# apache/datafusion

Hardware: AMD Instinct MI355X
Metric: tpch_q3_hash_join_rows_per_sec (higher is better)
Workload: dtype int64 keys / decimal128 payload; 1 GPU; INNER hash-join orders⋈lineitem on o_orderkey, TPC-H SF100, Q3 payload (o_orderdate,o_shippriority,l_orderkey,l_extendedprice,l_discount), device-resident inputs; build_rows=150000000, probe_rows=599960064, output_rows=599960064, join_table=rank_map, probe=single_pass_unordered, parallelism=single GPU, exchange=none

## Files before the change

datafusion_amd/csrc/internal.hpp:

```cpp
#pragma once
#include <atomic>
#include <hip/hip_runtime.h>

#include <chrono>
#include <cstdint>
#include <cstring>
#include <map>
#include <memory>
#include <mutex>
#include <stdexcept>
#include <string>
#include <thread>
#include <vector>

#include "../../include/dfgpu.h"

namespace dfgpu {

struct Error : std::runtime_error {
  using std::runtime_error::runtime_error;
};

void set_last_error(const std::string& msg);

// ... 97 lines not shown
int64_t scan_upload_caches_bytes(int device);
Runtime& rt_of(int device);
void use_device(int device);
int current_device();
const std::vector<int>& initialised_devices();
void require_init();

struct ProfileScope {
  hipEvent_t a = nullptr, b = nullptr;
  const char* name;
  int64_t bytes;
  ProfileScope(const char* name, int64_t algorithmic_bytes);
  ~ProfileScope();
};

struct DevBuf {
  void* ptr = nullptr;
  size_t bytes = 0;
  Runtime* owner = nullptr;
  std::shared_ptr<void> foreign;
  std::atomic<uint64_t> hint{0};
  std::atomic<uint64_t> all_hit_hint{0};
  explicit DevBuf(size_t n);
  DevBuf(void* p, size_t n, std::shared_ptr<void> keep_alive) : ptr(p), bytes(n), foreign(std::move(keep_alive)) {}
  ~DevBuf();
  DevBuf(const DevBuf&) = delete;
  DevBuf& operator=(const DevBuf&) = delete;
  template <typename T>
  T* as() const { return reinterpret_cast<T*>(ptr); }
};
using BufPtr = std::shared_ptr<DevBuf>;
inline BufPtr make_buf(size_t bytes) { return std::make_shared<DevBuf>(bytes ? bytes : 1); }
BufPtr make_zero_buf(size_t bytes);

void d2h(void* dst, const void* src, size_t n);
extern std::atomic<int64_t> g_pinned_driver_allocs, g_pinned_driver_ns;
void* pinned_alloc(size_t n);
void pinned_release(void* p);
void* stage_alloc(size_t n);
template <class T> struct StageAllocator {
  using value_type = T;
  StageAllocator() = default;
  template <class U> StageAllocator(const StageAllocator<U>&) {}
  T* allocate(size_t n) { return static_cast<T*>(stage_alloc(n * sizeof(T))); }
  void deallocate(T* p, size_t) { pinned_release(p); }
  template <class U> void construct(U* p) noexcept { ::new ((void*)p) U; }
  template <class U, class... A> void construct(U* p, A&&... a) { ::new ((void*)p) U(std::forward<A>(a)...); }
  template <class U> bool operator==(const StageAllocator<U>&) const { return true; }
  template <class U> bool operator!=(const StageAllocator<U>&) const { return false; }
};
template <class T> using StageVec = std::vector<T, StageAllocator<T>>;
struct PinnedBuf {
  void* ptr = nullptr;
  size_t bytes = 0;
  explicit PinnedBuf(size_t n) : ptr(pinned_alloc(n ? n : 1)), bytes(n) {}
  ~PinnedBuf() { pinned_release(ptr); }
  PinnedBuf(const PinnedBuf&) = delete;
  PinnedBuf& operator=(const PinnedBuf&) = delete;
  template <class T> T* as() const { return reinterpret_cast<T*>(ptr); }
};
void h2d_async(void* dst, const void* src, size_t n);

inline int type_width(int t) {
  switch (t) {
    case DFGPU_INT32: case DFGPU_UINT32: case DFGPU_DATE32: return 4;
    case DFGPU_INT64: case DFGPU_UINT64: case DFGPU_FLOAT64: return 8;
// ... 166 lines not shown
```

datafusion_amd/csrc/join.hip:

```cpp
#include <thread>
#include <functional>
#include <cstdlib>

#include "device.hpp"
#include "internal.hpp"
#include "grouped.hpp"

namespace dfgpu {

Table compact_table(const Table& in, const std::vector<int>& cols, const uint64_t* mask, const uint64_t* mask_valid);
void pack_bytes_to_bitmap(const uint8_t* bytes, int64_t n, uint64_t* words);

enum TableKind : int { KIND_HASH = 0, KIND_ARRAY = 1, KIND_RANK = 2, KIND_RADIX = 3, KIND_FLAT = 4, KIND_FLAT16 = 5,
                       KIND_RETURNED = 6 };
template <int KIND> constexpr bool kind_is_flat() { return KIND == KIND_FLAT || KIND == KIND_FLAT16; }
template <int KIND> constexpr bool kind_is_direct() { return KIND == KIND_ARRAY || KIND == KIND_RANK; }

struct FlatLayout {
  int n;
  uint8_t off[MAX_KEYS];
  uint8_t width[MAX_KEYS];
  int8_t null_bit[MAX_KEYS];
};
constexpr double RANK_MAP_MIN_KEY_DENSITY = 1.0 / 256.0;
// ... 250 lines not shown
        const int head_lane = 63 - __builtin_clzll(heads & ((2ull << lane) - 1ull));
        const uint64_t before = __shfl(inc - v, head_lane, 64);
        if (ok && ((tails >> lane) & 1ull)) atomicOr(&bits[w], (unsigned long long)(inc - before));
      }
    }
    return;
  }
  const int64_t stride = (int64_t)gridDim.x * BLOCK;
  for (int64_t i0 = (int64_t)blockIdx.x * BLOCK + threadIdx.x; i0 < n; i0 += stride * BUILD_UNROLL) {
    uint64_t lo[BUILD_UNROLL];
    bool ok[BUILD_UNROLL];
#pragma unroll
    for (int j = 0; j < BUILD_UNROLL; j++) {
      int64_t i = i0 + j * stride;
      lo[j] = load_key<KT>(k, i < n ? i : n - 1);
    }
#pragma unroll
    for (int j = 0; j < BUILD_UNROLL; j++) {
      int64_t i = i0 + j * stride;
      ok[j] = i < n;
      if (HASV) ok[j] = ok[j] && bit_at(k.valid, i < n ? i : n - 1);
    }
#pragma unroll
    for (int j = 0; j < BUILD_UNROLL; j++) {
      if (!ok[j]) continue;
      const uint64_t idx = lo[j] - offset;
      const unsigned long long bit = 1ull << (idx & 63);
      (void)__hip_atomic_fetch_or(&bits[idx >> 6], bit, __ATOMIC_RELAXED, __HIP_MEMORY_SCOPE_AGENT);
    }
  }
}
typedef unsigned long long rt_u64x2 __attribute__((ext_vector_type(2)));
typedef unsigned rt_u32x4 __attribute__((ext_vector_type(4)));
template <int KT>
__device__ __forceinline__ void load_keys4(const KeyCol& k, int64_t i0, uint64_t (&out)[4]) {
  if (KT == KT_I64 && ((uintptr_t)k.data & 15) == 0) {
    const rt_u64x2* p = reinterpret_cast<const rt_u64x2*>((const uint64_t*)k.data + i0);
    const rt_u64x2 a = __builtin_nontemporal_load(p), b = __builtin_nontemporal_load(p + 1);
    out[0] = a.x; out[1] = a.y; out[2] = b.x; out[3] = b.y;
  } else if ((KT == KT_I32 || KT == KT_U32) && ((uintptr_t)k.data & 15) == 0) {
    const rt_u32x4 a = __builtin_nontemporal_load(reinterpret_cast<const rt_u32x4*>((const uint32_t*)k.data + i0));
    out[0] = KT == KT_I32 ? (uint64_t)(int64_t)(int32_t)a.x : a.x;
    out[1] = KT == KT_I32 ? (uint64_t)(int64_t)(int32_t)a.y : a.y;
    out[2] = KT == KT_I32 ? (uint64_t)(int64_t)(int32_t)a.z : a.z;
    out[3] = KT == KT_I32 ? (uint64_t)(int64_t)(int32_t)a.w : a.w;
  } else {
#pragma unroll
    for (int j = 0; j < 4; j++) out[j] = load_key<KT, true>(k, i0 + j);
  }
}
constexpr int RT_ROWS = 4096;
constexpr int RT_WIN = 1024;
constexpr int RT_LANE_ROWS = 4;
constexpr int RT_CHUNK = WAVE * RT_LANE_ROWS;
constexpr int RT_STEPS = RT_ROWS / RT_CHUNK / (BLOCK / WAVE);
template <int KT, bool VERIFY>
__global__ __launch_bounds__(BLOCK) void k_rank_tab_onepass(KeyCol k, int64_t n, uint64_t offset, uint64_t range, ulonglong2* __restrict__ tab, int* __restrict__ flag) {
  __shared__ unsigned long long s_bits[RT_WIN];
  __shared__ unsigned s_first[RT_WIN];
  constexpr int WAVES = BLOCK / WAVE;
  const unsigned lane = lane_id();
  const int wv = threadIdx.x >> 6;
  const int64_t r0 = (int64_t)blockIdx.x * RT_ROWS;
  const int64_t r1 = r0 + RT_ROWS < n ? r0 + RT_ROWS : n;
  const uint64_t n_words = (range >> 6) + 1;
  uint64_t idx[RT_STEPS][RT_LANE_ROWS], pidx[RT_STEPS];
#pragma unroll
  for (int c = 0; c < RT_STEPS; c++) {
    const int64_t i0 = r0 + (int64_t)(c * WAVES + wv) * RT_CHUNK + lane * RT_LANE_ROWS;
    if (i0 + RT_LANE_ROWS <= n) {
      load_keys4<KT>(k, i0, idx[c]);
#pragma unroll
      for (int j = 0; j < RT_LANE_ROWS; j++) idx[c][j] -= offset;
    } else {
#pragma unroll
      for (int j = 0; j < RT_LANE_ROWS; j++) idx[c][j] = load_key<KT, true>(k, i0 + j < n ? i0 + j : n - 1) - offset;
    }
    pidx[c] = 0;
    if (VERIFY) pidx[c] = load_key<KT>(k, i0 < n ? (i0 > 0 ? i0 - 1 : 0) : n - 1) - offset;
  }
  const bool tail_lane = wv == WAVES - 1 && r1 + lane < n;
// ... 305 lines not shown
template <int KIND>
__device__ __forceinline__ uint32_t chain_head(const ProbeCtx& c, int64_t p) {
  if (kind_is_flat<KIND>()) {
    uint64_t k0, k1;
    if (!flat_pack(c.pkeys, c.flat_layout, p, c.null_equals_null != 0, k0, k1)) return 0u;
    return flat_find<KIND == KIND_FLAT16>(c.flat, c.flat_shift, c.flat_mask, k0, k1, c.force_collisions != 0);
  } else if (KIND != KIND_HASH) {
    const KeyCol& k = c.pkeys.c[0];
    if (k.valid && !bit_at(k.valid, p)) return 0;
    uint64_t lo, hi;
    load_words(k, p, lo, hi);
    uint64_t idx = lo - c.am_offset;
    if (idx >= c.am_size) return 0u;
    if (KIND == KIND_ARRAY) return c.heads[idx];
    const ulonglong2 e = c.rank_tab[idx >> 6];
    const uint64_t bits = e.x;
    if (!((bits >> (idx & 63)) & 1ull)) return 0u;
    const uint32_t rank = (uint32_t)e.y + (uint32_t)__popcll(bits & ((1ull << (idx & 63)) - 1ull));
    return (c.rank_perm ? c.rank_perm[rank] : rank) + 1u;
  } else {
    bool any_null;
    uint64_t h = hash_row(c.pkeys, p, SEED_JOIN, any_null);
    if (any_null && !c.null_equals_null) return 0;
    if (c.force_collisions) h = 0;
    return c.heads[h & c.hash_mask];
  }
}
template <int KIND>
__device__ __forceinline__ bool chain_match(const ProbeCtx& c, int64_t b, int64_t p) {
  if (KIND != KIND_HASH) return true;
  return keys_equal(c.bkeys, b, c.pkeys, p, c.null_equals_null);
}

template <int KIND, int KT, int N>
__device__ __forceinline__ void lookup_words(const ProbeCtx& c, int64_t w0, int64_t np, uint32_t (&m)[N], uint64_t* raw_keys = nullptr, uint4* rec16 = nullptr,
                                             uint32_t* key_rows = nullptr ) {
  const unsigned lane = lane_id();
  if (KIND == KIND_RETURNED) {
    uint32_t d[N];
    bool ok[N];
#pragma unroll
    for (int j = 0; j < N; j++) {
      const int64_t p = ((w0 + j) << 6) + lane;
      ok[j] = p < np;
      d[j] = c.ret_dest[ok[j] ? p : np - 1];
      if (c.row_mask) ok[j] = ok[j] && ((c.row_mask[w0 + j] >> lane) & 1ull);
    }
    if (rec16 && c.ret_R == 16) {
#pragma unroll
      for (int j = 0; j < N; j++) {
        ok[j] = ok[j] && d[j] != 0xFFFFFFFFu;
        rec16[j] = reinterpret_cast<const uint4*>(c.ret_rec)[ok[j] ? d[j] : 0u];
      }
#pragma unroll
      for (int j = 0; j < N; j++) m[j] = ok[j] ? rec16[j].x : 0u;
      return;
    }
#pragma unroll
    for (int j = 0; j < N; j++) {
      ok[j] = ok[j] && d[j] != 0xFFFFFFFFu;
      m[j] = *reinterpret_cast<const uint32_t*>(c.ret_rec + (uint64_t)(ok[j] ? d[j] : 0u) * (uint64_t)c.ret_R);
    }
#pragma unroll
    for (int j = 0; j < N; j++) m[j] = ok[j] ? m[j] : 0u;
    return;
  }
// ... 33 lines not shown
      int64_t p = ((w0 + j) << 6) + lane;
      const bool live = p < np && (!c.row_mask || ((c.row_mask[w0 + j] >> lane) & 1ull));
      m[j] = live ? chain_head<KIND>(c, p) : 0u;
    }
#pragma unroll
    for (int j = 0; j < N; j++) {
      int64_t p = ((w0 + j) << 6) + lane;
      while (m[j] && !chain_match<KIND>(c, (int64_t)m[j] - 1, p)) m[j] = c.next[m[j] - 1];
    }
    return;
  }
  const KeyCol& k = c.pkeys.c[0];
  uint64_t idx[N];
  bool ok[N];
#pragma unroll
  for (int j = 0; j < N; j++) {
    int64_t p = ((w0 + j) << 6) + lane;
    ok[j] = p < np;
    idx[j] = load_key<KT>(k, ok[j] ? p : np - 1);
    if (raw_keys) raw_keys[j] = idx[j];
    idx[j] -= c.am_offset;
    if (c.row_mask) ok[j] = ok[j] && ((c.row_mask[w0 + j] >> lane) & 1ull);
  }
  if (k.valid) {
    uint64_t vw[N];
#pragma unroll
    for (int j = 0; j < N; j++) {
      int64_t p = ((w0 + j) << 6) + lane;
      vw[j] = k.valid[(p < np ? p : np - 1) >> 6];
    }
#pragma unroll
    for (int j = 0; j < N; j++) ok[j] = ok[j] && ((vw[j] >> lane) & 1ull);
  }
#pragma unroll
  for (int j = 0; j < N; j++) {
    ok[j] = ok[j] && idx[j] < c.am_size;
    if (!ok[j]) idx[j] = 0;
  }
  if (KIND == KIND_ARRAY) {
#pragma unroll
    for (int j = 0; j < N; j++) m[j] = c.heads[idx[j]];
#pragma unroll
    for (int j = 0; j < N; j++) m[j] = ok[j] ? m[j] : 0u;
  } else {
    uint64_t bits[N], pre[N];
#pragma unroll
    for (int j = 0; j < N; j++) {
      const ulonglong2 e = c.rank_tab[idx[j] >> 6];
      bits[j] = e.x;
      pre[j] = e.y;
    }
#pragma unroll
    for (int j = 0; j < N; j++) {
      const bool hit = ok[j] && ((bits[j] >> (idx[j] & 63)) & 1ull);
      const uint32_t rank = (uint32_t)pre[j] + (uint32_t)__popcll(bits[j] & ((1ull << (idx[j] & 63)) - 1ull));
      m[j] = hit ? rank + 1u : 0u;
    }
    if (c.rank_perm) {
      uint32_t row[N];
#pragma unroll
      for (int j = 0; j < N; j++) row[j] = c.rank_perm[m[j] ? m[j] - 1 : 0u];
#pragma unroll
      for (int j = 0; j < N; j++) m[j] = m[j] ? row[j] + 1u : 0u;
    }
  }
}

template <int KIND, int KT, int N, bool NT = false>
__device__ __forceinline__ void hit_words(const ProbeCtx& c, int64_t w0, int64_t np, uint64_t (&word)[N], const bool* pre = nullptr, const uint64_t* keys_in = nullptr) {
  if (KIND != KIND_RANK) {
    uint32_t m[N];
    lookup_words<KIND, KT, N>(c, w0, np, m);
#pragma unroll
    for (int j = 0; j < N; j++) word[j] = ballot64(m[j] != 0);
    return;
  }
  const unsigned lane = lane_id();
  const KeyCol& k = c.pkeys.c[0];
  uint64_t idx[N];
  bool ok[N];
#pragma unroll
  for (int j = 0; j < N; j++) {
    const int64_t p = ((w0 + j) << 6) + lane;
    ok[j] = p < np;
    idx[j] = (keys_in ? keys_in[j] : load_key<KT, NT>(k, ok[j] ? p : np - 1)) - c.am_offset;
    if (pre) ok[j] = ok[j] && pre[j];
    else if (c.row_mask) ok[j] = ok[j] && ((c.row_mask[w0 + j] >> lane) & 1ull);
  }
  if (k.valid) {
    uint64_t vw[N];
#pragma unroll
    for (int j = 0; j < N; j++) {
      const int64_t p = ((w0 + j) << 6) + lane;
      vw[j] = k.valid[(p < np ? p : np - 1) >> 6];
    }
#pragma unroll
    for (int j = 0; j < N; j++) ok[j] = ok[j] && ((vw[j] >> lane) & 1ull);
  }
// ... 497 lines not shown
        }
        const int word_of_lane = lane >> 4;
#pragma unroll
        for (int q = 0; q < 4; q++) {
          const int from = (4 * lane + q) & 63;
#pragma unroll
          for (int jj = 0; jj < 4; jj++) {
            const uint32_t t = __shfl(v[jj], from);
            if (jj == word_of_lane) o[q] = t;
          }
        }
        const int64_t row0 = ((w0 + 4 * g) << 6) + 4 * (int64_t)lane;
        uint32_t* dst = reinterpret_cast<uint32_t*>(cols.dst[cidx]) + row0;
        if (row0 + 3 < np) {
          stream_store(reinterpret_cast<uint4*>(dst), make_uint4(o[0], o[1], o[2], o[3]));
        } else {
#pragma unroll
          for (int q = 0; q < 4; q++)
            if (row0 + q < np) dst[q] = o[q];
        }
      }
      continue;
    }
#pragma unroll
    for (int j = 0; j < W; j++) {
      const int64_t d = ((w0 + j) << 6) + lane;
      if (d >= np || !m[j]) continue;
      const int64_t s = (int64_t)m[j] - 1;
      switch (width) {
        case 16: jcopy_stream<uint4>(cols.src[cidx], cols.dst[cidx], s, d, false, true); break;
        case 8: jcopy_stream<uint64_t>(cols.src[cidx], cols.dst[cidx], s, d, false, true); break;
        case 1: jcopy_stream<uint8_t>(cols.src[cidx], cols.dst[cidx], s, d, false, true); break;
      }
    }
  }
}

constexpr int EL_WORDS = 128;
constexpr int EL_WORDS_SPARSE = 1024;
constexpr int EL_CAP = 8192;
template <int KIND, int KT, int EW>
__global__ __launch_bounds__(BLOCK) void k_join_emit_listed(ProbeCtx c, JoinCopyCols cols, int64_t np, const uint64_t* __restrict__ out_words,
                                                            const uint64_t* __restrict__ tile_prefix, int tiles_per_group) {
  static_assert(EW % BLOCK == 0 || BLOCK % EW == 0, "whole words per thread");
  static_assert(EW * 64 <= 65536, "a listed row is a 16-bit index into the group");
  constexpr int WPT = EW >= BLOCK ? EW / BLOCK : 1;
  __shared__ uint64_t s_word[EW];
  __shared__ uint32_t s_off[EW];
  __shared__ uint32_t s_wsum[BLOCK / WAVE];
  __shared__ uint16_t s_row[EL_CAP];
  const int64_t n_words = (np + 63) >> 6;
  const int64_t w_base = (int64_t)blockIdx.x * EW;
  const unsigned lane = lane_id();
  const int wv = threadIdx.x >> 6;
  uint64_t w[WPT];
  uint32_t cnt = 0;
#pragma unroll
  for (int t = 0; t < WPT; t++) {
    const int i = (int)threadIdx.x * WPT + t;
    w[t] = (i < EW && w_base + i < n_words) ? out_words[w_base + i] : 0ull;
    cnt += (uint32_t)__popcll(w[t]);
  }
  const uint32_t inc = wave_inclusive_sum(cnt);
  if (lane == 63) s_wsum[wv] = inc;
#pragma unroll
  for (int t = 0; t < WPT; t++) {
// ... 1378 lines not shown
  if (fused_ok && fused_mode == FUSED_UNORDERED && np > (1 << 22) && !unclustered && !in_grouped_probe && !returned) {
    int64_t row_bytes = key_bytes / std::max<int64_t>(np, 1) + out_row_bytes;
    for (int c : pout) {
      bool is_key = false;
      for (int k : pk) is_key |= k == c;
      if (!is_key) row_bytes += type_width(probe.cols[c].field.type);
    }
    if (row_bytes * (FUSED_W * BLOCK) < 12 * 6000) fused_mode = FUSED_PLACED;
  }
  const bool one_match_path = np > 0 && (probe_side_only || fast_inner);
  const bool use_fused_now = use_fused;
  const bool pred_in_counts = lazy != nullptr && use_fused && listed && fused_mode == FUSED_PLACED && !returned && (kind == KIND_RANK || kind == KIND_ARRAY);
  if (!pred_in_counts) need_mask();
  if (row_mask || pred_in_counts) {
    DFGPU_CHECK(mask_consumed != nullptr, "probe row mask without a fallback");
    *mask_consumed = use_fused || one_match_path;
    if (!*mask_consumed) return Table{};
    ctx.row_mask = row_mask;
  }
  const bool listed_flavour = use_fused_now && listed && fused_mode == FUSED_PLACED && kind == KIND_RANK;
  if (!listed_flavour) need_tab();
  if (use_fused_now && fused_mode != FUSED_PLACED) {
    size_t free_b = 0, total_b = 0;
    DFGPU_HIP(hipMemGetInfo(&free_b, &total_b));
    DFGPU_CHECK(np * out_row_bytes <= (int64_t)free_b + r.cached, "single-pass probe: the np-row upper bound of the output does not fit in HBM");
  }

  if (use_fused_now) {
    const int64_t tile_words = (int64_t)FUSED_W * (BLOCK / WAVE);
    const int64_t n_tiles = (n_words + tile_words - 1) / tile_words;
    const int invert = join_type == DFGPU_JOIN_RIGHT_ANTI;
    ctx.row_mask = row_mask;
    BufPtr state = fused_mode == FUSED_LOOKBACK ? make_zero_buf((size_t)n_tiles * 8) : nullptr;
    BufPtr ctl = make_zero_buf(sizeof(FusedCtl));
    BufPtr out_words;
    int64_t n_alloc = np;
    static thread_local bool no_speculation = false;
    DevBuf* hit_hint = nullptr;
    uint64_t hit_tag = 0;
    auto probe_again_counted = [&](hipEvent_t ea, hipEvent_t eb) {
      if (hit_hint) hit_hint->all_hit_hint.store(hit_tag, std::memory_order_relaxed);
      if (r.profiling) {
        std::lock_guard<std::mutex> lk(r.mu);
        r.recs.push_back(Runtime::Rec{"join_probe_speculation_missed", ea, eb, 0, std::this_thread::get_id()});
      }
      {
        std::lock_guard<std::mutex> lk(jt.mu);
        jt.info.probe_rows -= np;
      }
      out = Table{};
      no_speculation = true;
      Table again;
      try {
        again = join_probe(jt, probe, pk, join_type, bout_in, pout, row_mask, mask_consumed);
      } catch (...) {
        no_speculation = false;
        throw;
      }
      no_speculation = false;
      return again;
    };
    bool speculate = false;
    const bool spec_kind = kind == KIND_RANK || kind == KIND_ARRAY || kind == KIND_FLAT || kind == KIND_FLAT16;
    const bool may_sample = !row_mask && !lazy && !invert && !no_speculation && spec_kind && np >= option_int("join.share_probe_min_rows", 1 << 22);
    const bool share_wanted = option_on("join.share_probe", true) && jt.probe_mode != 2 && !returned && (fast_inner || join_type == DFGPU_JOIN_RIGHT_SEMI);
    if (returned_all_hit && !no_speculation) {
      speculate = true;
// ... 1 lines not shown
      hit_hint = probe.cols[(size_t)pk[0]].data.get();
      hit_tag = all_hit_tag(jt, probe, pk, kind);
      const uint64_t h = hit_hint->all_hit_hint.load(std::memory_order_relaxed);
      if ((h & ~1ull) == hit_tag) {
        speculate = (h & 1ull) != 0;
      } else {
        constexpr int S = 1024;
        BufPtr miss = make_zero_buf(4);
        with_kind_and_key(kind, ctx.pkeys.c[0].type, [&](auto kd, auto kt) {
          k_sample_all_hit<decltype(kd)::value, decltype(kt)::value><<<S * WAVE / BLOCK, BLOCK, 0, r.stream>>>(ctx, np, std::max<int64_t>(1, n_words / S), S, miss->as<int>());
        });
        DFGPU_HIP(hipGetLastError());
        int m = 0;
        d2h(&m, miss->ptr, 4);
        speculate = m == 0;
        hit_hint->all_hit_hint.store(hit_tag | (speculate ? 1ull : 0ull), std::memory_order_relaxed);
      }
    }
    if (speculate && share_wanted && !returned_all_hit) {
      need_tab();
      JoinCopyCols jc{};
      jc.key_col = -1;
      int64_t bytes = key_bytes;
      for (int c : bout) {
        const Column& sc = jt.build.cols[c];
        out.cols.push_back(alloc_like(sc, np));
        jc.src[jc.n] = sc.ptr();
        jc.dst[jc.n] = out.cols.back().data->ptr;
        jc.width[jc.n] = type_width(sc.field.type);
        bytes += (jt.build.nrows + np) * jc.width[jc.n];
        jc.n++;
      }
      jc.n_build = jc.n;
      hipEvent_t ea = nullptr, eb = nullptr, sa = nullptr, sb = nullptr;
      if (r.profiling) {
        for (hipEvent_t* e : {&ea, &eb, &sa, &sb}) DFGPU_HIP(hipEventCreate(e));
        DFGPU_HIP(hipEventRecord(ea, r.stream));
      }
      with_kind_and_key(kind, ctx.pkeys.c[0].type, [&](auto kd, auto kt) {
        constexpr int K = decltype(kd)::value, T = decltype(kt)::value;
        if constexpr (K == KIND_RANK || K == KIND_ARRAY || K == KIND_FLAT || K == KIND_FLAT16) {
          const int64_t waves = (n_words + SHARED_W - 1) / SHARED_W;
          const unsigned g = (unsigned)((waves + BLOCK / WAVE - 1) / (BLOCK / WAVE));
          k_join_probe_shared<K, T, SHARED_W><<<g, BLOCK, 0, r.stream>>>(ctx, jc, np, ctl->as<FusedCtl>());
        }
      });
      DFGPU_HIP(hipGetLastError());
      if (r.profiling) {
        DFGPU_HIP(hipEventRecord(eb, r.stream));
        DFGPU_HIP(hipEventRecord(sa, r.stream));
        DFGPU_HIP(hipEventRecord(sb, r.stream));
      }
      unsigned missed = 0;
      d2h(&missed, &ctl->as<FusedCtl>()->ticket, 4);
      if (missed) {
        if (r.profiling) {
          DFGPU_HIP(hipEventDestroy(sa));
          DFGPU_HIP(hipEventDestroy(sb));
        }
        return probe_again_counted(ea, eb);
      }
      for (int c : pout) {
        out.cols.push_back(probe.cols[c]);
        out.cols.back().length = np;
      }
      if (r.profiling) {
        std::lock_guard<std::mutex> lk(r.mu);
        r.recs.push_back(Runtime::Rec{want_single ? "join_probe_fused" : "join_probe_placed", ea, eb, bytes, std::this_thread::get_id()});
        r.recs.push_back(Runtime::Rec{"join_probe_shared_columns", sa, sb, 0, std::this_thread::get_id()});
      }
      out.nrows = np;
      jt.info.output_rows += out.nrows;
      return out;
    }
    speculate = speculate && fused_mode == FUSED_PLACED && !listed;
    if (fused_mode == FUSED_PLACED && !speculate) {
      BufPtr counts = make_buf((size_t)n_tiles * 4);
      state = make_buf((size_t)(n_tiles + 1) * 8);
      if (listed) out_words = make_buf((size_t)n_words * 8);
      if (kind == KIND_RANK) need_bits();
      {
        ProfileScope ps("join_probe_tile_counts", key_bytes + (pred_in_counts ? np * lazy->pred_bytes_per_row : 0));
        with_kind_and_key(kind, ctx.pkeys.c[0].type, [&](auto kd, auto kt) {
          constexpr int K = decltype(kd)::value, T = decltype(kt)::value;
          if constexpr (kind_is_direct<K>()) {
            const bool nt = option_on("join.counts_nt", true);
            if (pred_in_counts) {
              if (nt) k_join_tile_counts<K, T, FUSED_W, true, true><<<(unsigned)n_tiles, BLOCK, 0, r.stream>>>(ctx, np, invert, nullptr, counts->as<uint32_t>(), out_words->as<uint64_t>(), lazy->pred);
              else k_join_tile_counts<K, T, FUSED_W, true><<<(unsigned)n_tiles, BLOCK, 0, r.stream>>>(ctx, np, invert, nullptr, counts->as<uint32_t>(), out_words->as<uint64_t>(), lazy->pred);
              return;
            }
            if (nt) {
              k_join_tile_counts<K, T, FUSED_W, false, true><<<(unsigned)n_tiles, BLOCK, 0, r.stream>>>(ctx, np, invert, row_mask, counts->as<uint32_t>(), out_words ? out_words->as<uint64_t>() : nullptr);
              return;
            }
          }
          k_join_tile_counts<K, T, FUSED_W><<<(unsigned)n_tiles, BLOCK, 0, r.stream>>>(
              ctx, np, invert, row_mask, counts->as<uint32_t>(), out_words ? out_words->as<uint64_t>() : nullptr);
        });
        DFGPU_HIP(hipGetLastError());
      }
      scan_u32(counts->as<uint32_t>(), n_tiles, state->as<uint64_t>());
      n_alloc = (int64_t)read_u64(state->as<uint64_t>() + n_tiles);
      listed = listed && n_alloc * 4 <= np;
      if (!listed) need_tab();
      if (pred_in_counts && !listed) {
        row_mask = out_words->as<uint64_t>();
        ctx.row_mask = row_mask;
// ... 905 lines not shown
```

datafusion_amd/csrc/runtime.hip:

```cpp
#include "internal.hpp"

#include <chrono>
#include <algorithm>
#include <cstring>
#include <atomic>

namespace dfgpu {

static thread_local std::string g_last_error;
void set_last_error(const std::string& msg) { g_last_error = msg; }

static std::mutex g_devices_mu;
static std::vector<std::unique_ptr<Runtime>> g_runtimes;
static std::vector<int> g_initialised;
static Runtime g_uninitialised;
static thread_local int t_device = -1;
static thread_local int t_hip_device = -1;

const std::vector<int>& initialised_devices() { return g_initialised; }
int current_device() {
  if (t_device >= 0) return t_device;
  return g_initialised.empty() ? -1 : g_initialised[0];
}
Runtime& rt_of(int device) {
// ... 45 lines not shown
    auto it = g_options.find(name);
    if (it != g_options.end()) {
      out = it->second;
      return true;
    }
  }
  return env_option(name, out);
}
int64_t option_int(const char* name, int64_t dflt) {
  std::string v;
  return find_option(name, v) && !v.empty() ? (int64_t)std::atoll(v.c_str()) : dflt;
}
bool option_on(const char* name, bool dflt) {
  std::string v;
  if (!find_option(name, v) || v.empty()) return dflt;
  return !(v == "0" || v == "off" || v == "false");
}
std::string option_str(const char* name, const char* dflt) {
  std::string v;
  return find_option(name, v) ? v : std::string(dflt ? dflt : "");
}
bool trace_on(const char* what) {
  const char* e = std::getenv("DFGPU_TRACE");
  if (!e || !*e) return false;
  return std::strstr(e, what) != nullptr || std::strstr(e, "all") != nullptr;
}


struct ThreadDevice {
  hipStream_t stream = nullptr;
  uint64_t generation = 0;
  bool borrowed = false;
  std::vector<std::pair<size_t, void*>> pending;
};
struct SpareStreams {
  std::mutex mu;
  std::map<int, std::vector<hipStream_t>> by_device;
};
static SpareStreams& spare_streams() {
  static SpareStreams* s = new SpareStreams();
  return *s;
}
static std::atomic<bool> g_multi_thread{false};
static std::atomic<std::thread::id> g_first_thread{};
struct ThreadState {
  std::vector<ThreadDevice> dev;
  ~ThreadState() {
    for (size_t d = 0; d < dev.size(); d++) {
      ThreadDevice& td = dev[d];
      if (!td.pending.empty() && d < g_runtimes.size() && g_runtimes[d]) {
        if (td.stream) (void)hipStreamSynchronize(td.stream);
        std::lock_guard<std::mutex> lk(g_runtimes[d]->mu);
        for (auto& b : td.pending) {
          g_runtimes[d]->free_blocks.emplace(b.first, b.second);
          g_runtimes[d]->cached += (int64_t)b.first;
        }
      }
      if (td.stream && td.borrowed) {
        std::lock_guard<std::mutex> lk(spare_streams().mu);
        spare_streams().by_device[(int)d].push_back(td.stream);
      }
    }
  }
};
static thread_local ThreadState t_state;
static ThreadDevice& thread_device(int device) {
  if ((int)t_state.dev.size() <= device) t_state.dev.resize((size_t)device + 1);
  return t_state.dev[(size_t)device];
}

StreamRef::operator hipStream_t() const { return r ? r->thread_stream() : nullptr; }

hipStream_t Runtime::thread_stream() {
  if (!initialised) return nullptr;
  ThreadDevice& td = thread_device(device);
  if (td.stream && td.generation == generation) return td.stream;
  if (td.stream && !td.borrowed) td.stream = nullptr;
  td.generation = generation;
  if (td.stream) return td.stream;
  const std::thread::id me = std::this_thread::get_id();
  std::thread::id none{};
  if (g_first_thread.compare_exchange_strong(none, me) || g_first_thread.load() == me) {
    td.stream = first_stream;
    return td.stream;
  }
  if (!g_multi_thread.exchange(true)) (void)hipDeviceSynchronize();
  {
    std::lock_guard<std::mutex> lk(spare_streams().mu);
    auto& spare = spare_streams().by_device[device];
    if (!spare.empty()) {
      td.stream = spare.back();
      spare.pop_back();
    }
  }
  if (!td.stream) DFGPU_HIP(hipStreamCreateWithFlags(&td.stream, hipStreamNonBlocking));
  td.borrowed = true;
  return td.stream;
}

void call_epilogue() noexcept {
  if (!g_multi_thread.load(std::memory_order_relaxed)) return;
  for (size_t d = 0; d < t_state.dev.size(); d++) {
    ThreadDevice& td = t_state.dev[d];
// ... 77 lines not shown
  {
    std::lock_guard<std::mutex> lk(mu);
    auto it = live.find(p);
    if (it == live.end()) return;
    cap = it->second;
    live.erase(it);
    in_use -= (int64_t)cap;
    if (!g_multi_thread.load(std::memory_order_seq_cst)) {
      free_blocks.emplace(cap, p);
      cached += (int64_t)cap;
      return;
    }
  }
  thread_device(device).pending.emplace_back(cap, p);
}

void Runtime::trim() {
  scan_upload_caches_drop(device);
  call_epilogue();
  std::multimap<size_t, void*> blocks;
  {
    std::lock_guard<std::mutex> lk(mu);
    blocks.swap(free_blocks);
    cached = 0;
  }
  if (blocks.empty()) return;
  (void)hipDeviceSynchronize();
  for (auto& kv : blocks) (void)hipFree(kv.second);
}

DevBuf::DevBuf(size_t n) : bytes(n), owner(&rt()) { ptr = owner->alloc(n); }
DevBuf::~DevBuf() {
  if (owner) owner->free(ptr);
}

BufPtr make_zero_buf(size_t bytes) {
  BufPtr b = make_buf(bytes);
  DFGPU_HIP(hipMemsetAsync(b->ptr, 0, bytes ? bytes : 1, rt().stream));
  return b;
}

void d2h(void* dst, const void* src, size_t n) {
  constexpr size_t PIN = 64 << 10;
  static thread_local void* t_pin = nullptr;
  if (n <= PIN && option_on("runtime.pinned_readback", true)) {
    if (!t_pin && hipHostMalloc(&t_pin, PIN, hipHostMallocDefault) != hipSuccess) {
      (void)hipGetLastError();
      t_pin = nullptr;
    }
    if (t_pin) {
      DFGPU_HIP(hipMemcpyAsync(t_pin, src, n, hipMemcpyDeviceToHost, rt().stream));
      DFGPU_HIP(hipStreamSynchronize(rt().stream));
      std::memcpy(dst, t_pin, n);
      return;
    }
  }
  DFGPU_HIP(hipMemcpyAsync(dst, src, n, hipMemcpyDeviceToHost, rt().stream));
  DFGPU_HIP(hipStreamSynchronize(rt().stream));
}
void h2d_async(void* dst, const void* src, size_t n) {
  DFGPU_HIP(hipMemcpyAsync(dst, src, n, hipMemcpyHostToDevice, rt().stream));
}
uint64_t read_u64(const uint64_t* dev) {
  uint64_t v = 0;
  d2h(&v, dev, 8);
  return v;
// ... 171 lines not shown
        if (a == b) continue;
        int can = 0;
        if (hipDeviceCanAccessPeer(&can, a, b) == hipSuccess && can) {
          (void)hipSetDevice(a);
          hipError_t pe = hipDeviceEnablePeerAccess(b, 0);
          if (pe != hipSuccess) (void)hipGetLastError();
        }
      }
    if (t_device < 0) t_device = g_initialised[0];
    DFGPU_HIP(hipSetDevice(t_device));
    t_hip_device = t_device;
  });
}

int dfgpu_set_device(int device) {
  return guarded([&] { use_device(device); });
}
int dfgpu_get_device(int* out) {
  return guarded([&] {
    require_init();
    *out = current_device();
  });
}

int dfgpu_shutdown(void) {
  return guarded([&] {
    std::lock_guard<std::mutex> lk(g_devices_mu);
    for (int d : g_initialised) {
      Runtime& r = *g_runtimes[d];
      (void)hipSetDevice(d);
      r.collect();
      r.trim();
      r.initialised = false;
      (void)hipStreamDestroy(r.first_stream);
      r.first_stream = nullptr;
      {
        std::lock_guard<std::mutex> sl(spare_streams().mu);
        for (hipStream_t s : spare_streams().by_device[d]) (void)hipStreamDestroy(s);
        spare_streams().by_device[d].clear();
      }
    }
    g_initialised.clear();
    t_device = t_hip_device = -1;
  });
}

int dfgpu_sync(void) {
  return guarded([&] {
    require_init();
    if (g_multi_thread.load()) DFGPU_HIP(hipDeviceSynchronize());
    else DFGPU_HIP(hipStreamSynchronize(rt().stream));
  });
}

void* dfgpu_stream(void) { return (void*)(hipStream_t)rt().stream; }

int dfgpu_mem_stats(int64_t* in_use, int64_t* cached, int64_t* peak) {
  return guarded([&] {
    Runtime& r = rt();
    std::lock_guard<std::mutex> lk(r.mu);
    if (in_use) *in_use = r.in_use;
    if (cached) *cached = r.cached;
    if (peak) *peak = r.peak;
  });
}
int dfgpu_mem_trim(void) {
  return guarded([&] { rt().trim(); });
}

namespace {
struct Reservation {
// ... 115 lines not shown
```

Before: 356.2 billion rows/s.

## Add four-rows-per-lane direct-address probe kernel and reuse per-stream control word

Adds a new probe kernel for rank/array join tables in which each lane loads four consecutive keys with 16-byte vector loads, does a batched direct lookup, and gathers build columns with wide streaming stores. The shared lookup logic is factored into a helper. The per-call zeroed control buffer (a memset plus allocation) is replaced by a persistent per-stream control block that is only cleared after a miss. The wider per-lane work raises register use and changes the gather access pattern, and the persistent control word relies on being reset correctly after each miss.

```diff
diff --git a/datafusion_amd/csrc/internal.hpp b/datafusion_amd/csrc/internal.hpp
--- a/datafusion_amd/csrc/internal.hpp
+++ b/datafusion_amd/csrc/internal.hpp
@@ -153,6 +153,9 @@
 using BufPtr = std::shared_ptr<DevBuf>;
 inline BufPtr make_buf(size_t bytes) { return std::make_shared<DevBuf>(bytes ? bytes : 1); }
 BufPtr make_zero_buf(size_t bytes);
+constexpr size_t STREAM_CTL_BYTES = 256;
+void* stream_ctl();
+void stream_ctl_clear();
 
 void d2h(void* dst, const void* src, size_t n);
 extern std::atomic<int64_t> g_pinned_driver_allocs, g_pinned_driver_ns;
diff --git a/datafusion_amd/csrc/join.hip b/datafusion_amd/csrc/join.hip
--- a/datafusion_amd/csrc/join.hip
+++ b/datafusion_amd/csrc/join.hip
@@ -306,21 +306,22 @@
 }
 typedef unsigned long long rt_u64x2 __attribute__((ext_vector_type(2)));
 typedef unsigned rt_u32x4 __attribute__((ext_vector_type(4)));
-template <int KT>
+template <int KT, bool NT = true>
 __device__ __forceinline__ void load_keys4(const KeyCol& k, int64_t i0, uint64_t (&out)[4]) {
   if (KT == KT_I64 && ((uintptr_t)k.data & 15) == 0) {
     const rt_u64x2* p = reinterpret_cast<const rt_u64x2*>((const uint64_t*)k.data + i0);
-    const rt_u64x2 a = __builtin_nontemporal_load(p), b = __builtin_nontemporal_load(p + 1);
+    const rt_u64x2 a = NT ? __builtin_nontemporal_load(p) : p[0], b = NT ? __builtin_nontemporal_load(p + 1) : p[1];
     out[0] = a.x; out[1] = a.y; out[2] = b.x; out[3] = b.y;
   } else if ((KT == KT_I32 || KT == KT_U32) && ((uintptr_t)k.data & 15) == 0) {
-    const rt_u32x4 a = __builtin_nontemporal_load(reinterpret_cast<const rt_u32x4*>((const uint32_t*)k.data + i0));
+    const rt_u32x4* p = reinterpret_cast<const rt_u32x4*>((const uint32_t*)k.data + i0);
+    const rt_u32x4 a = NT ? __builtin_nontemporal_load(p) : p[0];
     out[0] = KT == KT_I32 ? (uint64_t)(int64_t)(int32_t)a.x : a.x;
     out[1] = KT == KT_I32 ? (uint64_t)(int64_t)(int32_t)a.y : a.y;
     out[2] = KT == KT_I32 ? (uint64_t)(int64_t)(int32_t)a.z : a.z;
     out[3] = KT == KT_I32 ? (uint64_t)(int64_t)(int32_t)a.w : a.w;
   } else {
 #pragma unroll
-    for (int j = 0; j < 4; j++) out[j] = load_key<KT, true>(k, i0 + j);
+    for (int j = 0; j < 4; j++) out[j] = load_key<KT, NT>(k, i0 + j);
   }
 }
 constexpr int RT_ROWS = 4096;
@@ -692,6 +693,42 @@
   return keys_equal(c.bkeys, b, c.pkeys, p, c.null_equals_null);
 }
 
+template <int KIND, int N>
+__device__ __forceinline__ void direct_lookup(const ProbeCtx& c, uint64_t (&idx)[N], bool (&ok)[N], uint32_t (&m)[N]) {
+#pragma unroll
+  for (int j = 0; j < N; j++) {
+    ok[j] = ok[j] && idx[j] < c.am_size;
+    if (!ok[j]) idx[j] = 0;
+  }
+  if (KIND == KIND_ARRAY) {
+#pragma unroll
+    for (int j = 0; j < N; j++) m[j] = c.heads[idx[j]];
+#pragma unroll
+    for (int j = 0; j < N; j++) m[j] = ok[j] ? m[j] : 0u;
+  } else {
+    uint64_t bits[N], pre[N];
+#pragma unroll
+    for (int j = 0; j < N; j++) {
+      const ulonglong2 e = c.rank_tab[idx[j] >> 6];
+      bits[j] = e.x;
+      pre[j] = e.y;
+    }
+#pragma unroll
+    for (int j = 0; j < N; j++) {
+      const bool hit = ok[j] && ((bits[j] >> (idx[j] & 63)) & 1ull);
+      const uint32_t rank = (uint32_t)pre[j] + (uint32_t)__popcll(bits[j] & ((1ull << (idx[j] & 63)) - 1ull));
+      m[j] = hit ? rank + 1u : 0u;
+    }
+    if (c.rank_perm) {
+      uint32_t row[N];
+#pragma unroll
+      for (int j = 0; j < N; j++) row[j] = c.rank_perm[m[j] ? m[j] - 1 : 0u];
+#pragma unroll
+      for (int j = 0; j < N; j++) m[j] = m[j] ? row[j] + 1u : 0u;
+    }
+  }
+}
+
 template <int KIND, int KT, int N>
 __device__ __forceinline__ void lookup_words(const ProbeCtx& c, int64_t w0, int64_t np, uint32_t (&m)[N], uint64_t* raw_keys = nullptr, uint4* rec16 = nullptr,
                                              uint32_t* key_rows = nullptr ) {
@@ -791,38 +828,7 @@
 #pragma unroll
     for (int j = 0; j < N; j++) ok[j] = ok[j] && ((vw[j] >> lane) & 1ull);
   }
-#pragma unroll
-  for (int j = 0; j < N; j++) {
-    ok[j] = ok[j] && idx[j] < c.am_size;
-    if (!ok[j]) idx[j] = 0;
-  }
-  if (KIND == KIND_ARRAY) {
-#pragma unroll
-    for (int j = 0; j < N; j++) m[j] = c.heads[idx[j]];
-#pragma unroll
-    for (int j = 0; j < N; j++) m[j] = ok[j] ? m[j] : 0u;
-  } else {
-    uint64_t bits[N], pre[N];
-#pragma unroll
-    for (int j = 0; j < N; j++) {
-      const ulonglong2 e = c.rank_tab[idx[j] >> 6];
-      bits[j] = e.x;
-      pre[j] = e.y;
-    }
-#pragma unroll
-    for (int j = 0; j < N; j++) {
-      const bool hit = ok[j] && ((bits[j] >> (idx[j] & 63)) & 1ull);
-      const uint32_t rank = (uint32_t)pre[j] + (uint32_t)__popcll(bits[j] & ((1ull << (idx[j] & 63)) - 1ull));
-      m[j] = hit ? rank + 1u : 0u;
-    }
-    if (c.rank_perm) {
-      uint32_t row[N];
-#pragma unroll
-      for (int j = 0; j < N; j++) row[j] = c.rank_perm[m[j] ? m[j] - 1 : 0u];
-#pragma unroll
-      for (int j = 0; j < N; j++) m[j] = m[j] ? row[j] + 1u : 0u;
-    }
-  }
+  direct_lookup<KIND, N>(c, idx, ok, m);
 }
 
 template <int KIND, int KT, int N, bool NT = false>
@@ -1386,6 +1392,111 @@
         case 8: jcopy_stream<uint64_t>(cols.src[cidx], cols.dst[cidx], s, d, false, true); break;
         case 1: jcopy_stream<uint8_t>(cols.src[cidx], cols.dst[cidx], s, d, false, true); break;
       }
+    }
+  }
+}
+
+template <typename T, int G, int GG>
+__device__ __forceinline__ void shared4_column(const void* __restrict__ src, void* __restrict__ dst, const uint32_t (&m)[4 * G], int64_t r0, int64_t np) {
+  static_assert(G % GG == 0, "whole rounds");
+  const T* s = reinterpret_cast<const T*>(src);
+#pragma unroll
+  for (int g0 = 0; g0 < G; g0 += GG) {
+    T v[GG][4];
+#pragma unroll
+    for (int g = 0; g < GG; g++)
+#pragma unroll
+      for (int q = 0; q < 4; q++) {
+        const uint32_t id = m[4 * (g0 + g) + q];
+        if (id) v[g][q] = s[id - 1];
+        else v[g][q] = T{};
+      }
+#pragma unroll
+    for (int g = 0; g < GG; g++) {
+      const int64_t row0 = r0 + (int64_t)(g0 + g) * (4 * WAVE) + 4 * (int64_t)lane_id();
+      T* d = reinterpret_cast<T*>(dst) + row0;
+      if (row0 + 3 < np) {
+        if constexpr (sizeof(T) == 4) {
+          stream_store(reinterpret_cast<uint4*>(d), make_uint4(v[g][0], v[g][1], v[g][2], v[g][3]));
+        } else if constexpr (sizeof(T) == 8) {
+          stream_store(reinterpret_cast<uint4*>(d), make_uint4((uint32_t)v[g][0], (uint32_t)(v[g][0] >> 32), (uint32_t)v[g][1], (uint32_t)(v[g][1] >> 32)));
+          stream_store(reinterpret_cast<uint4*>(d) + 1, make_uint4((uint32_t)v[g][2], (uint32_t)(v[g][2] >> 32), (uint32_t)v[g][3], (uint32_t)(v[g][3] >> 32)));
+        } else if constexpr (sizeof(T) == 16) {
+#pragma unroll
+          for (int q = 0; q < 4; q++) stream_store(d + q, v[g][q]);
+        } else {
+          stream_store(reinterpret_cast<uint32_t*>(d), (uint32_t)v[g][0] | ((uint32_t)v[g][1] << 8) | ((uint32_t)v[g][2] << 16) | ((uint32_t)v[g][3] << 24));
+        }
+      } else {
+#pragma unroll
+        for (int q = 0; q < 4; q++)
+          if (row0 + q < np) d[q] = v[g][q];
+      }
+    }
+  }
+}
+
+#ifndef DFGPU_ROWS4_GROUPS
+#define DFGPU_ROWS4_GROUPS 2
+#endif
+#ifndef DFGPU_ROWS4_NT
+#define DFGPU_ROWS4_NT 0
+#endif
+constexpr int SHARED4_G = DFGPU_ROWS4_GROUPS;
+constexpr int SHARED4_GROUP_ROWS = 4 * WAVE;
+template <int KIND, int KT, int G, bool NT>
+__global__ __launch_bounds__(BLOCK) void k_join_probe_shared4(ProbeCtx c, JoinCopyCols cols, int64_t np, FusedCtl* __restrict__ ctl) {
+  static_assert(KIND == KIND_RANK || KIND == KIND_ARRAY, "direct-address kinds");
+  static_assert(KT == KT_I64 || KT == KT_I32, "keys that load_keys4 takes 16 bytes at a time");
+  constexpr int N = 4 * G;
+  const unsigned lane = lane_id();
+  const int64_t r0 = ((((int64_t)blockIdx.x * BLOCK) + threadIdx.x) >> 6) * (G * SHARED4_GROUP_ROWS);
+  if (r0 >= np) return;
+  const KeyCol& k = c.pkeys.c[0];
+  uint64_t idx[N];
+  bool ok[N];
+#pragma unroll
+  for (int g = 0; g < G; g++) {
+    const int64_t row0 = r0 + g * SHARED4_GROUP_ROWS + 4 * (int64_t)lane;
+    uint64_t k4[4] = {0, 0, 0, 0};
+    if (row0 + 3 < np) {
+      load_keys4<KT, NT>(k, row0, k4);
+    } else {
+#pragma unroll
+      for (int q = 0; q < 4; q++)
+        if (row0 + q < np) k4[q] = load_key<KT>(k, row0 + q);
+    }
+#pragma unroll
+    for (int q = 0; q < 4; q++) {
+      idx[4 * g + q] = k4[q] - c.am_offset;
+      ok[4 * g + q] = row0 + q < np;
+    }
+  }
+  if (k.valid) {
+    uint64_t vw[G];
+#pragma unroll
+    for (int g = 0; g < G; g++) {
+      const int64_t row0 = r0 + g * SHARED4_GROUP_ROWS + 4 * (int64_t)lane;
+      vw[g] = row0 < np ? k.valid[row0 >> 6] : 0ull;
+    }
+#pragma unroll
+    for (int j = 0; j < N; j++) ok[j] = ok[j] && ((vw[j >> 2] >> ((4 * lane + (j & 3)) & 63)) & 1ull);
+  }
+  uint32_t m[N];
+  direct_lookup<KIND, N>(c, idx, ok, m);
+  bool missed = false;
+#pragma unroll
+  for (int j = 0; j < N; j++) missed |= (r0 + (j >> 2) * SHARED4_GROUP_ROWS + 4 * (int64_t)lane + (j & 3)) < np && m[j] == 0;
+  const uint64_t miss_word = ballot64(missed);
+  if (miss_word && lane == (unsigned)__builtin_ctzll(miss_word)) ctl->ticket = 1u;
+  for (int cidx = 0; cidx < cols.n_build; cidx++) {
+    const void* src = cols.src[cidx];
+    void* dst = cols.dst[cidx];
+    switch (cols.width[cidx]) {
+      case 4: shared4_column<uint32_t, G, G>(src, dst, m, r0, np); break;
+      case 8: shared4_column<uint64_t, G, G>(src, dst, m, r0, np); break;
+      case 16: shared4_column<uint4, G, 1>(src, dst, m, r0, np); break;
+      case 1: shared4_column<uint8_t, G, G>(src, dst, m, r0, np); break;
     }
   }
 }
@@ -2830,7 +2941,6 @@
     const int invert = join_type == DFGPU_JOIN_RIGHT_ANTI;
     ctx.row_mask = row_mask;
     BufPtr state = fused_mode == FUSED_LOOKBACK ? make_zero_buf((size_t)n_tiles * 8) : nullptr;
-    BufPtr ctl = make_zero_buf(sizeof(FusedCtl));
     BufPtr out_words;
     int64_t n_alloc = np;
     static thread_local bool no_speculation = false;
@@ -2898,17 +3008,34 @@
         jc.n++;
       }
       jc.n_build = jc.n;
-      hipEvent_t ea = nullptr, eb = nullptr, sa = nullptr, sb = nullptr;
+      const int key_type = ctx.pkeys.c[0].type;
+      const bool rows4 = (kind == KIND_RANK || kind == KIND_ARRAY) && (key_type == DFGPU_INT64 || key_type == DFGPU_INT32 || key_type == DFGPU_DATE32) &&
+                         ((uintptr_t)ctx.pkeys.c[0].data & 15) == 0 && option_on("join.share_probe_rows4", true);
+      static_assert(sizeof(FusedCtl) <= STREAM_CTL_BYTES, "the shared probe's control word lives in the stream's control block");
+      const bool ctl_once = option_on("join.share_probe_ctl_once", true);
+      BufPtr ctl_fresh = ctl_once ? nullptr : make_zero_buf(sizeof(FusedCtl));
+      FusedCtl* const ctl = ctl_once ? reinterpret_cast<FusedCtl*>(stream_ctl()) : ctl_fresh->as<FusedCtl>();
+      hipEvent_t ea = nullptr, eb = nullptr, sa = nullptr, sb = nullptr, ra = nullptr, rb = nullptr;
       if (r.profiling) {
         for (hipEvent_t* e : {&ea, &eb, &sa, &sb}) DFGPU_HIP(hipEventCreate(e));
+        if (rows4)
+          for (hipEvent_t* e : {&ra, &rb}) DFGPU_HIP(hipEventCreate(e));
         DFGPU_HIP(hipEventRecord(ea, r.stream));
       }
       with_kind_and_key(kind, ctx.pkeys.c[0].type, [&](auto kd, auto kt) {
         constexpr int K = decltype(kd)::value, T = decltype(kt)::value;
+        if constexpr ((K == KIND_RANK || K == KIND_ARRAY) && (T == KT_I64 || T == KT_I32)) {
+          if (rows4) {
+            const int64_t waves = (np + SHARED4_G * SHARED4_GROUP_ROWS - 1) / (SHARED4_G * SHARED4_GROUP_ROWS);
+            const unsigned g = (unsigned)((waves + BLOCK / WAVE - 1) / (BLOCK / WAVE));
+            k_join_probe_shared4<K, T, SHARED4_G, DFGPU_ROWS4_NT != 0><<<g, BLOCK, 0, r.stream>>>(ctx, jc, np, ctl);
+            return;
+          }
+        }
         if constexpr (K == KIND_RANK || K == KIND_ARRAY || K == KIND_FLAT || K == KIND_FLAT16) {
           const int64_t waves = (n_words + SHARED_W - 1) / SHARED_W;
           const unsigned g = (unsigned)((waves + BLOCK / WAVE - 1) / (BLOCK / WAVE));
-          k_join_probe_shared<K, T, SHARED_W><<<g, BLOCK, 0, r.stream>>>(ctx, jc, np, ctl->as<FusedCtl>());
+          k_join_probe_shared<K, T, SHARED_W><<<g, BLOCK, 0, r.stream>>>(ctx, jc, np, ctl);
         }
       });
       DFGPU_HIP(hipGetLastError());
@@ -2916,13 +3043,18 @@
         DFGPU_HIP(hipEventRecord(eb, r.stream));
         DFGPU_HIP(hipEventRecord(sa, r.stream));
         DFGPU_HIP(hipEventRecord(sb, r.stream));
+        if (rows4) {
+          DFGPU_HIP(hipEventRecord(ra, r.stream));
+          DFGPU_HIP(hipEventRecord(rb, r.stream));
+        }
       }
       unsigned missed = 0;
-      d2h(&missed, &ctl->as<FusedCtl>()->ticket, 4);
+      d2h(&missed, &ctl->ticket, 4);
       if (missed) {
+        if (ctl_once) stream_ctl_clear();
         if (r.profiling) {
-          DFGPU_HIP(hipEventDestroy(sa));
-          DFGPU_HIP(hipEventDestroy(sb));
+          for (hipEvent_t e : {sa, sb, ra, rb})
+            if (e) DFGPU_HIP(hipEventDestroy(e));
         }
         return probe_again_counted(ea, eb);
       }
@@ -2934,12 +3066,14 @@
         std::lock_guard<std::mutex> lk(r.mu);
         r.recs.push_back(Runtime::Rec{want_single ? "join_probe_fused" : "join_probe_placed", ea, eb, bytes, std::this_thread::get_id()});
         r.recs.push_back(Runtime::Rec{"join_probe_shared_columns", sa, sb, 0, std::this_thread::get_id()});
+        if (rows4) r.recs.push_back(Runtime::Rec{"join_probe_shared_rows4", ra, rb, 0, std::this_thread::get_id()});
       }
       out.nrows = np;
       jt.info.output_rows += out.nrows;
       return out;
     }
     speculate = speculate && fused_mode == FUSED_PLACED && !listed;
+    BufPtr ctl = make_zero_buf(sizeof(FusedCtl));
     if (fused_mode == FUSED_PLACED && !speculate) {
       BufPtr counts = make_buf((size_t)n_tiles * 4);
       state = make_buf((size_t)(n_tiles + 1) * 8);
diff --git a/datafusion_amd/csrc/runtime.hip b/datafusion_amd/csrc/runtime.hip
--- a/datafusion_amd/csrc/runtime.hip
+++ b/datafusion_amd/csrc/runtime.hip
@@ -101,6 +101,9 @@
   uint64_t generation = 0;
   bool borrowed = false;
   std::vector<std::pair<size_t, void*>> pending;
+  void* ctl = nullptr;
+  hipStream_t ctl_stream = nullptr;
+  uint64_t ctl_generation = 0;
 };
 struct SpareStreams {
   std::mutex mu;
@@ -138,6 +141,26 @@
   return t_state.dev[(size_t)device];
 }
 
+struct StreamCtls {
+  std::mutex mu;
+  std::map<hipStream_t, void*> by_stream;
+};
+static StreamCtls& stream_ctls() {
+  static StreamCtls* s = new StreamCtls();
+  return *s;
+}
+static void stream_ctl_release(hipStream_t s) {
+  void* p = nullptr;
+  {
+    std::lock_guard<std::mutex> lk(stream_ctls().mu);
+    auto it = stream_ctls().by_stream.find(s);
+    if (it == stream_ctls().by_stream.end()) return;
+    p = it->second;
+    stream_ctls().by_stream.erase(it);
+  }
+  (void)hipFree(p);
+}
+
 StreamRef::operator hipStream_t() const { return r ? r->thread_stream() : nullptr; }
 
 hipStream_t Runtime::thread_stream() {
@@ -281,6 +304,38 @@
 DevBuf::DevBuf(size_t n) : bytes(n), owner(&rt()) { ptr = owner->alloc(n); }
 DevBuf::~DevBuf() {
   if (owner) owner->free(ptr);
+}
+
+void* stream_ctl() {
+  Runtime& r = rt();
+  const hipStream_t s = r.stream;
+  DFGPU_CHECK(s != nullptr, "stream_ctl: the device is not initialised");
+  ThreadDevice& td = thread_device(r.device);
+  if (td.ctl && td.ctl_stream == s && td.ctl_generation == r.generation) return td.ctl;
+  void* p = nullptr;
+  {
+    std::lock_guard<std::mutex> lk(stream_ctls().mu);
+    auto it = stream_ctls().by_stream.find(s);
+    if (it != stream_ctls().by_stream.end()) p = it->second;
+  }
+  if (!p) {
+    DFGPU_HIP(hipMalloc(&p, STREAM_CTL_BYTES));
+    hipError_t e = hipMemsetAsync(p, 0, STREAM_CTL_BYTES, s);
+    if (e != hipSuccess) {
+      (void)hipFree(p);
+      DFGPU_HIP(e);
+    }
+    std::lock_guard<std::mutex> lk(stream_ctls().mu);
+    stream_ctls().by_stream[s] = p;
+  }
+  td.ctl = p;
+  td.ctl_stream = s;
+  td.ctl_generation = r.generation;
+  return p;
+}
+void stream_ctl_clear() {
+  void* p = stream_ctl();
+  DFGPU_HIP(hipMemsetAsync(p, 0, STREAM_CTL_BYTES, rt().stream));
 }
 
 BufPtr make_zero_buf(size_t bytes) {
@@ -518,11 +573,15 @@
       r.collect();
       r.trim();
       r.initialised = false;
+      stream_ctl_release(r.first_stream);
       (void)hipStreamDestroy(r.first_stream);
       r.first_stream = nullptr;
       {
         std::lock_guard<std::mutex> sl(spare_streams().mu);
-        for (hipStream_t s : spare_streams().by_device[d]) (void)hipStreamDestroy(s);
+        for (hipStream_t s : spare_streams().by_device[d]) {
+          stream_ctl_release(s);
+          (void)hipStreamDestroy(s);
+        }
         spare_streams().by_device[d].clear();
       }
     }
```

New measurement: 349.4 billion rows/s. 1.9% lower.
